# TencentYoutuResearch/ImageMatching-OETR

Hardware: AMD Instinct MI355X
Metric: image-pairs/sec @640x640 (OETR hot path: feature correlation + overlap regression, features resident in HBM) (higher is better)
Workload: dtype f32 (3xf16-split operands, fp32 accumulate); 1 GPU; BASELINE configs[1]: batch=8 pairs/GPU, 640x640 -> 20x20 tokens/image, C=256, 8 enc + 2 dec layers, f32_split_f16; pairs_per_gpu=8, global_pairs=8, streams=3, world_size=1, gpu_max_hw_queues=4, encoder_tile_rows=64, tail_mode=direct form (throughput setting for overlapped streams), parallelism=pairs sharded over 1 rank(s); all-gather of boxes only

## Files before the change

### imagematching_oetr_amd/csrc/api.hip

```cpp
#include <math.h>
#include <stdlib.h>
#include <string.h>

#include <atomic>
#include <string>
#include <vector>

#include "../../include/oetr_hip.h"
#include "../../include/oetr_tail_share.h"
#include "common.h"

using namespace oetr;

constexpr int OETR_PREREDUCE_MIN_TOKENS = 768;
constexpr int OETR_DIRECT_TAIL_MIN_ROWS = 16000;

namespace {

thread_local std::string g_err;

oetr_status fail(oetr_status st, const std::string& msg) {
  g_err = msg;
  return st;
}
// ... 124 lines not shown
  size_t dev_floats = 0;
  EncLayerDev enc[OETR_N_ENC];
  DecKVDev dkv;
  DecLayerDev dec[OETR_N_DEC];
  const float* qe[2];
  const float *dec_tgt1, *dec_q0, *dec_qkv1;
  HeadsDev heads;
};

struct oetr_neck_ctx {
  oetr_trace* trace = nullptr;
  int device = 0;
  int num_cus = 256;
  int conv_rows = 0;
  float* dev = nullptr;
  const f32x4 *proj_wh[2], *proj_wl[2];
  const float *proj_b, *ln_w, *ln_b;
  const f32x4 *conv_wh[3], *conv_wl[3];
  const f32x4 *conv_wh_rw[3], *conv_wl_rw[3];
  int conv_kernel = 0;
  const float* conv_b[3];
  const f32x4 *out_wh, *out_wl;
  const float* out_b;
};

namespace {

#ifdef OETR_PHASE_TIMING
long long* g_tbuf = nullptr;
#endif

struct Workspace {
  float *x, *qp, *pos, *kvp[2], *ksp[2], *att0, *z0, *dkv1, *dks1, *conv_out, *gn_part, *sm_part, *hs,
      *logits, *cxy, *tlbr, *convp, *kbuf[2], *vt[2], *kvr, *ksr;
  uint32_t* flags;
  size_t bytes;
};

bool make_geom(int n, int hf1, int wf1, int hf2, int wf2, Geom* g) {
  if (n <= 0 || hf1 <= 0 || wf1 <= 0 || hf2 <= 0 || wf2 <= 0) return false;
  const long L1 = (long)hf1 * wf1, L2 = (long)hf2 * wf2;
  if (L1 > OETR_MAX_TOKENS || L2 > OETR_MAX_TOKENS) return false;
  if ((long)n * (L1 + L2) > (1L << 30) / C) return false;
  g->N = n;
  g->L[0] = (int)L1; g->L[1] = (int)L2;
  g->hf[0] = hf1; g->wf[0] = wf1; g->hf[1] = hf2; g->wf[1] = wf2;
  g->nt[0] = (g->L[0] + TM - 1) / TM; g->nt[1] = (g->L[1] + TM - 1) / TM;
  g->row0[0] = 0; g->row0[1] = n * g->L[0];
  g->prow0[0] = 0; g->prow0[1] = g->L[0];
  g->tile0[0] = 0; g->tile0[1] = n * g->nt[0];
  g->ntiles = n * (g->nt[0] + g->nt[1]);
  g->rows = n * (g->L[0] + g->L[1]);
  return true;
}

int encoder_tile_rows(const oetr_ctx* h, const Geom& g) {
  if (!gm_half(h->mode) || h->attn_full) return TM;
  const int want = h->enc_tile;
  if (want == TM || want == 64) return want;
  return g.ntiles > h->num_cus ? 64 : TM;
}
Geom encoder_geom(const Geom& g, int rows) {
  Geom e = g;
  for (int i = 0; i < 2; ++i) e.nt[i] = (g.L[i] + rows - 1) / rows;
  e.tile0[0] = 0; e.tile0[1] = g.N * e.nt[0];
  e.ntiles = g.N * (e.nt[0] + e.nt[1]);
  return e;
}

Workspace carve(const Geom& g, void* base, bool attn_full = false) {
  Workspace w;
  size_t off = 0;
  auto take = [&](size_t floats) {
    float* p = base ? reinterpret_cast<float*>(static_cast<char*>(base) + off) : nullptr;
    off += (floats * sizeof(float) + 255) & ~size_t(255);
    return p;
  };
  const size_t rows = g.rows, nt = g.ntiles;
  w.flags = reinterpret_cast<uint32_t*>(take(OETR_WORKSPACE_STATUS_BYTES / sizeof(float)));
  w.x = take(rows * C);
  w.qp = take((rows + (size_t)2 * g.N * 64) * C);
  w.pos = take((size_t)(g.L[0] + g.L[1]) * C);
  for (int i = 0; i < 2; ++i) { w.kvp[i] = take(nt * KV_FLOATS); w.ksp[i] = take(nt * C); }
  w.att0 = take(nt * C); w.z0 = take(nt * NH);
  w.dkv1 = take(nt * KV_FLOATS); w.dks1 = take(nt * C);
  w.conv_out = take(rows * C);
  w.gn_part = take(nt * 32 * 2);
  w.sm_part = take(nt * 4);
  w.hs = take((size_t)2 * g.N * C);
  w.logits = take(rows);
  w.cxy = take((size_t)2 * g.N * 2);
  w.tlbr = take((size_t)2 * g.N * 4);
  w.convp = take((size_t)9 * rows * C);
  w.kvr = take((size_t)2 * g.N * KV_FLOATS);
  w.ksr = take((size_t)2 * g.N * C);
  for (int i = 0; i < 2; ++i) {
    w.kbuf[i] = attn_full ? take(rows * C) : nullptr;
    w.vt[i] = attn_full ? take((size_t)g.N * C * TM * (g.nt[0] + g.nt[1])) : nullptr;
  }
  w.bytes = off;
  return w;
}

oetr_status check_ws(const Geom& g, void* ws, size_t ws_bytes, Workspace* out, bool attn_full = false) {
  if (!ws) return fail(OETR_ERR_WORKSPACE, "workspace is NULL");
  if (reinterpret_cast<uintptr_t>(ws) & 255)
    return fail(OETR_ERR_WORKSPACE, "workspace must be 256-byte aligned");
  *out = carve(g, ws, attn_full);
  if (out->bytes > ws_bytes)
    return fail(OETR_ERR_WORKSPACE, "workspace too small: need " + std::to_string(out->bytes) +
                                        " bytes, got " + std::to_string(ws_bytes));
  return OETR_OK;
}

HeatLaunch heat_launch(const oetr_ctx* h, const Geom& g, const Workspace& w, const float* mem1,
                       const float* mem2, const float* hs1, const float* hs2, float* cxy1,
                       float* cxy2, int img_h1, int img_h2) {
  HeatLaunch p;
  p.g = g;
  p.w = h->heads;
  p.mem[0] = mem1; p.mem[1] = mem2;
  p.hs[0] = hs1; p.hs[1] = hs2;
  p.conv_out = w.conv_out;
  p.gn_part = w.gn_part;
  p.sm_part = w.sm_part;
  p.logits = w.logits;
  p.cxy[0] = cxy1; p.cxy[1] = cxy2;
  p.img_h[0] = img_h1; p.img_h[1] = img_h2;
  p.tlbr[0] = p.tlbr[1] = nullptr;
  p.box[0] = p.box[1] = nullptr;
  p.img_w[0] = p.img_w[1] = 0;
  p.flags = w.flags;
  p.publish = nullptr;
  p.force_staged_conv = h->tail_mode == 3;
  p.convp_units = 9;
  p.mask[0] = p.mask[1] = nullptr;
  return p;
}

oetr_status check_masks(const oetr_ctx* h, const float* mask1, const float* mask2, bool encoder) {
  if (!mask1 && !mask2) return OETR_OK;
  if (!mask1 || !mask2) return fail(OETR_ERR_BAD_ARG, "masks: pass both mask1 and mask2, or neither");
  if (encoder && ((h->mode != GM_SPLIT && h->mode != GM_F32) || h->attn_full))
    return fail(OETR_ERR_UNSUPPORTED, "masks: built for OETR_DTYPE_F32_SPLIT_F16, OETR_DTYPE_F32_SPLIT_QK16 and OETR_DTYPE_F32 with linear attention "
                                      "(the reference's FullAttention turns a masked query row into NaN, "
                                      "linear_attention.py:74-81)");
  return OETR_OK;
}

struct Scoped {
  oetr_trace* t; hipStream_t s; int slot;
  Scoped(oetr_trace* tr, hipStream_t s_, int kid) : t(tr), s(s_), slot(-1) {
    if (!t) return;
    if (2 * (t->used + 1) > (int)t->ev.size()) { t->dropped++; t = nullptr; return; }
    slot = t->used++;
    t->kid[slot] = kid;
    (void)hipEventRecord(t->ev[2 * slot], s);
  }
  ~Scoped() { if (t) (void)hipEventRecord(t->ev[2 * slot + 1], s); }
};
#define TRACED(h, s, kid, expr)            \
  do {                                     \
    Scoped sc__((h)->trace, s, kid);       \
    HIP_TRY(expr);                         \
  } while (0)

DecLaunch dec_launch(const oetr_ctx* h, const Geom& g, const Workspace& w, bool beside_convp = false) {
  DecLaunch d;
  d.g = encoder_geom(g, encoder_tile_rows(h, g));
  for (int i = 0; i < 2; ++i) { d.layer[i] = h->dec[i]; d.qe[i] = h->qe[i]; }
  d.tgt1 = h->dec_tgt1; d.qkv1 = h->dec_qkv1;
  d.att0_part = w.att0; d.z0_part = w.z0; d.dkv1 = w.dkv1; d.dks1 = w.dks1;
  d.hs = w.hs;
  const int images = 2 * g.N;
  bool fits = images <= DEC_SPLIT_MAX_IMAGES && images * DEC_SPLIT_K * 4 <= h->num_cus;
  d.convp_units = 9;
  if (fits && beside_convp) {
    if (gm_half(h->mode)) {
      const int units = 9 * g.N * ((g.L[0] + RT - 1) / RT + (g.L[1] + RT - 1) / RT);
      const int avail = h->num_cus - images * DEC_SPLIT_K;
      const int upi = std::max(3, (units + avail - 1) / avail);
      fits = upi <= 9;
      if (fits) d.convp_units = upi;
    } else {
      fits = images * DEC_SPLIT_K + g.ntiles <= h->num_cus;
    }
  }
  if (h->dec_split == DEC_SPLIT_K && d.convp_units == 9 && beside_convp && gm_half(h->mode)) d.convp_units = 3;
  d.ksplit = (h->dec_split == DEC_SPLIT_K || (h->dec_split == 0 && fits)) && images <= DEC_SPLIT_MAX_IMAGES
                 ? DEC_SPLIT_K : 1;
  d.flags = w.flags;
  d.xch_epoch = w.flags + STATUS_EPOCH_WORD;
  d.xch = reinterpret_cast<unsigned long long*>(reinterpret_cast<char*>(w.flags) + STATUS_XCH_OFFSET);
  d.tbuf = nullptr;
  d.dbg = 0;
  if (d.ksplit == DEC_SPLIT_K && h->dec_fault) { d.dbg = DEC_DBG_FAULT; h->dec_fault = 0; }
#ifdef OETR_PHASE_TIMING
  d.tbuf = g_tbuf ? g_tbuf + 16 * 4096 : nullptr;
#endif
  return d;
}

oetr_status run_correlation(oetr_ctx* h, const Geom& g, const Workspace& w, const float* feat1,
                            const float* feat2, const float* pos1, const float* pos2,
                            int enc_layers, hipStream_t s, bool with_decoder = true,
                            bool resident = false, const float* mask1 = nullptr,
// ... 355 lines not shown
  if (!make_geom(n_pairs, hf1, wf1, hf2, wf2, &g))
    return fail(OETR_ERR_BAD_SHAPE, "invalid shape: need N>0 and 1 <= hf*wf <= " +
                                        std::to_string(OETR_MAX_TOKENS));
  if (full && (img_h1 < hf1 || img_h2 < hf2 || img_w1 <= 0 || img_w2 <= 0))
    return fail(OETR_ERR_BAD_SHAPE, "image size smaller than the token grid");
  Workspace w;
  oetr_status rc = check_ws(g, workspace, workspace_bytes, &w, h->attn_full);
  if (rc) return rc;
  hipStream_t s = static_cast<hipStream_t>(stream);
  rc = run_correlation(h, g, w, feat1, feat2, pos1, pos2, enc_layers, s, false, resident,
                       mask1, mask2);
  if (rc) return rc;
  const size_t r1 = (size_t)g.N * g.L[0], r2 = (size_t)g.N * g.L[1];
  if (st) {
    if ((rc = copy_out(st->memory1, w.x, r1 * C, s))) return rc;
    if ((rc = copy_out(st->memory2, w.x + r1 * C, r2 * C, s))) return rc;
  }
  if (!full) return OETR_OK;
  const float* hs1 = w.hs;
  const float* hs2 = w.hs + (size_t)g.N * C;
  float* cxy1 = w.cxy;
  float* cxy2 = w.cxy + 2 * g.N;
  float* tl1 = w.tlbr;
  float* tl2 = w.tlbr + 4 * g.N;
  HeatLaunch hp = heat_launch(h, g, w, w.x, w.x + r1 * C, hs1, hs2, cxy1, cxy2, img_h1, img_h2);
  hp.tlbr[0] = tl1; hp.tlbr[1] = tl2;
  hp.mask[0] = mask1; hp.mask[1] = mask2;
  hp.box[0] = box1; hp.box[1] = box2;
  hp.img_w[0] = img_w1; hp.img_w[1] = img_w2;
  hp.publish = publish;
  const bool direct = h->mode == GM_SPLIT &&
                      (h->tail_mode >= 2 || (h->tail_mode == 0 && g.rows >= OETR_DIRECT_TAIL_MIN_ROWS));
  if (direct) {
    TRACED(h, s, K_DECODER, launch_decoder(dec_launch(h, g, w), s));
    TRACED(h, s, K_HEAT_CONV, launch_heat_conv64(hp, h->mode, s));
  } else {
    TRACED(h, s, K_DEC_CONVP, launch_decoder_convp(dec_launch(h, g, w, true), hp, w.convp, h->mode, s));
    TRACED(h, s, K_HEAT_COMBINE, launch_heat_combine(hp, w.convp, s));
  }
  TRACED(h, s, K_HEAT_FINAL, launch_heat_final(hp, s));
  if (st) {
    if ((rc = copy_out(st->hs1, hs1, (size_t)g.N * C, s))) return rc;
    if ((rc = copy_out(st->hs2, hs2, (size_t)g.N * C, s))) return rc;
    if ((rc = copy_out(st->logits1, w.logits, r1, s))) return rc;
    if ((rc = copy_out(st->logits2, w.logits + r1, r2, s))) return rc;
    if ((rc = copy_out(st->cxy1, cxy1, 2 * g.N, s))) return rc;
    if ((rc = copy_out(st->cxy2, cxy2, 2 * g.N, s))) return rc;
    if ((rc = copy_out(st->tlbr1, tl1, 4 * g.N, s))) return rc;
    if ((rc = copy_out(st->tlbr2, tl2, 4 * g.N, s))) return rc;
  }
  return OETR_OK;
}
}

oetr_status oetr_forward_stages(oetr_handle h, const float* feat1, const float* feat2,
                                const float* pos1, const float* pos2, int n_pairs, int hf1,
                                int wf1, int hf2, int wf2, int img_h1, int img_w1, int img_h2,
                                int img_w2, void* workspace, size_t workspace_bytes,
                                float* box1, float* box2, const oetr_stage_outputs* st,
                                void* stream) {
  return forward_impl(h, feat1, feat2, pos1, pos2, n_pairs, hf1, wf1, hf2, wf2, img_h1, img_w1,
                      img_h2, img_w2, workspace, workspace_bytes, box1, box2, st, stream, false);
}

oetr_status oetr_forward_masked(oetr_handle h, const float* feat1, const float* feat2,
                                const float* pos1, const float* pos2, const float* mask1,
                                const float* mask2, int n_pairs, int hf1, int wf1, int hf2, int wf2,
// ... 653 lines not shown

oetr_status oetr_trace_summary(oetr_trace_handle t, int* n_kernels,
                               const char* names[OETR_TRACE_MAX_KERNELS],
                               int launches[OETR_TRACE_MAX_KERNELS],
                               float total_ms[OETR_TRACE_MAX_KERNELS]) {
  if (!t || !n_kernels || !names || !launches || !total_ms)
    return fail(OETR_ERR_BAD_ARG, "oetr_trace_summary: NULL argument");
  static_assert(K_COUNT <= OETR_TRACE_MAX_KERNELS, "raise OETR_TRACE_MAX_KERNELS");
  for (int i = 0; i < K_COUNT; ++i) { names[i] = kKernelNames[i]; launches[i] = 0; total_ms[i] = 0.f; }
  for (int i = 0; i < t->used; ++i) {
    HIP_TRY(hipEventSynchronize(t->ev[2 * i + 1]));
    float ms = 0.f;
    HIP_TRY(hipEventElapsedTime(&ms, t->ev[2 * i], t->ev[2 * i + 1]));
    launches[t->kid[i]]++;
    total_ms[t->kid[i]] += ms;
  }
  *n_kernels = K_COUNT;
  const int dropped = t->dropped;
  t->used = 0;
  t->dropped = 0;
  if (dropped) return fail(OETR_ERR_BAD_ARG, std::to_string(dropped) + " launches not traced: pool too small");
  return OETR_OK;
}

#ifdef OETR_PHASE_TIMING
int oetr_debug_read_tbuf(long long* host, int n_blocks) {
  if (!g_tbuf) return 1;
  return hipMemcpy(host, g_tbuf, sizeof(long long) * 16 * n_blocks, hipMemcpyDeviceToHost) != hipSuccess;
}
int oetr_debug_read_tbuf_decoder(long long* host, int n_blocks) {
  if (!g_tbuf) return 1;
  return hipMemcpy(host, g_tbuf + 16 * 4096, sizeof(long long) * 16 * n_blocks, hipMemcpyDeviceToHost) != hipSuccess;
}
#endif

}
```

### imagematching_oetr_amd/csrc/common.h

```cpp
#pragma once
#include <hip/hip_runtime.h>
#include <stdint.h>

#include <string>
#include <type_traits>

#include "../../include/oetr_hip.h"

namespace oetr {

constexpr int C = 256;
constexpr int NH = 8;
constexpr int HD = 32;
constexpr int FF = 512;
constexpr int TM = 32;
constexpr int LDA = C + 4;
constexpr int LDH = FF + 4;
constexpr int NTHREADS = 256;
constexpr int KV_FLOATS = NH * HD * HD;
constexpr float LN_EPS = 1e-5f;
constexpr float ATTN_EPS = 1e-6f;
constexpr int MAX_TOKENS = 10000;


// ... 839 lines not shown
  long long* tbuf;
  uint32_t* flags;
  const float* feat_nchw[2];
  const float* pos_nchw[2];
  float* pos_out;
  const float* mask[2];
};

hipError_t launch_encoder(const EncLaunch& p, bool has_b, int tail, int mode, hipStream_t s);
int encoder_workgroups(const EncLaunch& p, int mode);
hipError_t launch_kv_reduce(const Geom& g, const float* kvp, const float* ksp, float* kvr, float* ksr,
                            hipStream_t s);

struct MhaDev {
  const float *wq_t, *wk_t, *wv_t, *wm_t;
  const float *bq, *bk, *bv;
};
struct DecLayerDev {
  MhaDev self_attn, cross;
  const float *w1_t, *w2_t;
  const float *n1w, *n1b, *n2w, *n2b, *n3w, *n3b;
};
struct DecLaunch {
  Geom g;
  DecLayerDev layer[2];
  const float* qe[2];
  const float* tgt1;
  const float* qkv1;
  const float* att0_part;
  const float* z0_part;
  const float* dkv1;
  const float* dks1;
  float* hs;
  int convp_units;
  int ksplit;
  unsigned long long* xch;
  unsigned* xch_epoch;
  uint32_t* flags;
  long long* tbuf;
  int dbg;
};
struct DecConstLaunch {
  DecLayerDev layer[2];
  const float* qe[2];
  float *tgt1, *q0, *qkv1;
};
hipError_t launch_decoder_consts(const DecConstLaunch& p, hipStream_t s);
hipError_t launch_decoder(const DecLaunch& p, hipStream_t s);

struct HeadsDev {
  const f32x4* conv_w;
  const f32x4* conv_w_l;
  const float *conv_b, *gn_w, *gn_b, *out_w, *out_b;
  const float *tlbr0_t;
  const float *tlbr2_w, *tlbr2_b;
};
struct HeatLaunch {
  Geom g;
  HeadsDev w;
  const float* mem[2];
  const float* hs[2];
  float* conv_out;
  float* gn_part;
  float* sm_part;
  float* logits;
  float* cxy[2];
  int img_h[2];
  float* tlbr[2];
  float* box[2];
  int img_w[2];
  uint32_t* flags;
  uint32_t* publish;
  int force_staged_conv;
  int convp_units;
  const float* mask[2];
};
hipError_t launch_heat_conv(const HeatLaunch& p, int mode, hipStream_t s);
hipError_t launch_heat_conv64(const HeatLaunch& p, int mode, hipStream_t s);
hipError_t launch_decoder_convp(const DecLaunch& d, const HeatLaunch& h, float* P, int mode,
                                hipStream_t s);
hipError_t launch_heat_combine(const HeatLaunch& h, const float* P, hipStream_t s);
hipError_t launch_heat_final(const HeatLaunch& p, hipStream_t s);
hipError_t launch_size_regression(const HeadsDev& w, const float* hs1, const float* hs2,
                                  int n, float* tlbr1, float* tlbr2, hipStream_t s);
hipError_t launch_boxes(const float* cxy, const float* tlbr, int n, int max_h, int max_w,
                        float* box, hipStream_t s);
constexpr int BBC = 1024;
constexpr int NECK_MT = 256;
constexpr int NECK_PIX = 16;
constexpr int NECK_XROW = 2 * C;
constexpr int NECK_RW_MIN_WO = 16;
struct NeckGeom {
  int n_img, hb, wb, ho, wo;
  int HW;
  int rows_in;
  int M;
};
struct NeckProjLaunch {
  NeckGeom g;
  const float* bb;
  const f32x4 *wh[2], *wl[2];
  const float *bias, *ln_w, *ln_b;
  _Float16 *xh, *xl;
  uint32_t* flags;
};
struct NeckConvDesc {
  const f32x4 *wh, *wl;
  const f32x4 *wh_rw, *wl_rw;
// ... 41 lines not shown
```

### imagematching_oetr_amd/csrc/decoder.hip

```cpp
#include "common.h"
#include "conv_p.h"

namespace oetr {

constexpr int DEC_THREADS = 1024;

template <int K, int NOUT>
__device__ __forceinline__ void gemv_partial(const float* __restrict__ Wt, const float* x_s,
                                             float* part_s, int tid) {
  constexpr int NO4 = NOUT / 4;
  constexpr int KCH = DEC_THREADS / NO4;
  constexpr int KPER = K / KCH;
  constexpr int BATCH = KPER < 16 ? KPER : 16;
  const int kc = tid / NO4, o4 = tid % NO4;
  const f32x4* w = reinterpret_cast<const f32x4*>(Wt) + (size_t)kc * KPER * NO4 + o4;
  f32x4 acc = {0.f, 0.f, 0.f, 0.f};
#pragma unroll
  for (int i0 = 0; i0 < KPER; i0 += BATCH) {
    f32x4 wv[BATCH];
#pragma unroll
    for (int i = 0; i < BATCH; ++i) wv[i] = w[(size_t)(i0 + i) * NO4];
#pragma unroll
    for (int i = 0; i < BATCH; ++i) acc += wv[i] * x_s[kc * KPER + i0 + i];
  }
  *reinterpret_cast<f32x4*>(part_s + kc * NOUT + 4 * o4) = acc;
}
template <int K, int NOUT>
__device__ __forceinline__ float gemv_collect(const float* part_s, int o) {
  constexpr int KCH = DEC_THREADS / (NOUT / 4);
  float s = 0.f;
#pragma unroll
  for (int c = 0; c < KCH; ++c) s += part_s[c * NOUT + o];
  return s;
// ... 280 lines not shown
  if (tid < C) vq[tid] = elu1(gemv_get<T, C, C>(part_s, tid) + w1.cross.bq[tid]);
  __syncthreads();
  if (tid < C) {
    const int h = tid >> 5, v = tid & 31;
    float z = 0.f, s = 0.f;
#pragma unroll 4
    for (int d = 0; d < HD; ++d) {
      const float fq = vq[h * HD + d];
      z += fq * ksum[h * HD + d];
      s += fq * kv_s[(h * HD + d) * HD + v];
    }
    att[tid] = s * (1.0f / (z + ATTN_EPS)) * (float)L;
  }
  __syncthreads();
  PHASE_STAMP(p, 7);
  acc = zero4;
  gemv_stage<T, C, C>(w1.cross.wm_t, att, tid, wv, acc, [&] { gemv_issue<T, C, FF, 0>(w1.w1_t, tid, wv); });
  gemv_put<T, C, C>(acc, part_s, tid);
  __syncthreads();
  if (tid < C) tgt[tid] += gemv_get<T, C, C>(part_s, tid);
  __syncthreads();
  PHASE_STAMP(p, 8);
  ln_vec(tgt, w1.n3w, w1.n3b, t2, nullptr, nullptr, tid);
  acc = zero4;
  gemv_stage<T, C, FF>(w1.w1_t, t2, tid, wv, acc, [&] { gemv_issue<T, FF, C, 0>(w1.w2_t, tid, wv); });
  gemv_put<T, C, FF>(acc, part_s, tid);
  __syncthreads();
  for (int o = tid; o < FF; o += T) hdn_s[o] = fmaxf(gemv_get<T, C, FF>(part_s, o), 0.f);
  __syncthreads();
  acc = zero4;
  gemv_stage<T, FF, C>(w1.w2_t, hdn_s, tid, wv, acc, [] {});
  gemv_put<T, FF, C>(acc, part_s, tid);
  __syncthreads();
  if (tid < C) p.hs[(size_t)img * C + tid] = tgt[tid] + gemv_get<T, FF, C>(part_s, tid);
  PHASE_STAMP(p, 9);
}

constexpr int DEC_K = DEC_SPLIT_K;
constexpr int XCH_STAGES = DEC_SPLIT_EXCHANGES;
constexpr long long DEC_SPIN_LIMIT = 200000;

typedef __attribute__((address_space(1))) unsigned long long gu64;

struct DecSmem4 {
  static constexpr int KV = 0, PARTS = KV + 2 * HD * HD, VEC = PARTS + 3 * 2048, SLAB = VEC + 4 * C,
                       TOTAL = SLAB + 64 * 3 + 192 + 128;
};

template <int KS, int B0>
__device__ __forceinline__ void issue_rows(const float* __restrict__ Wt, int j, int tid, f32x4 (&w)[16]) {
  constexpr int KPER = KS / 8;
  const f32x4* src = reinterpret_cast<const f32x4*>(Wt) + (size_t)(j * KS + (tid >> 6) * KPER) * (C / 4) + (tid & 63);
#pragma unroll
  for (int i = 0; i < KPER; ++i) w[B0 + i] = src[i * (C / 4)];
  __builtin_amdgcn_sched_barrier(0);
}
template <int NS, int LD, int B0>
__device__ __forceinline__ void issue_cols(const float* __restrict__ Wt, int j, int tid, f32x4 (&w)[16]) {
  constexpr int NO4 = NS / 4, KCH = 512 / NO4, KPER = C / KCH;
  const f32x4* src = reinterpret_cast<const f32x4*>(Wt) + (size_t)((tid / NO4) * KPER) * (LD / 4) + j * NO4 + tid % NO4;
#pragma unroll
  for (int i = 0; i < KPER; ++i) w[B0 + i] = src[i * (LD / 4)];
  __builtin_amdgcn_sched_barrier(0);
}
template <int KS, int B0>
__device__ __forceinline__ void fma_rows(const f32x4 (&w)[16], const float* x_s, float* part_s, int tid) {
  constexpr int KPER = KS / 8;
  const int kc = tid >> 6;
// ... 173 lines not shown
  PHASE_STAMP(p, 5);
  fma_rows<64, 8>(wa, att, part_s, tid);
  issue_cols<128, FF, 0>(w1.w1_t, j, tid, wa);
  __syncthreads();
  if (tid < C) tgt[tid] += exchange_sum<false>(p, img, 2, j, tag, collect<8, C>(part_s, tid), tid, dead);
  __syncthreads();
  PHASE_STAMP(p, 6);
  ln_vec(tgt, w1.n2w, w1.n2b, t2, qe, qk, tid);
  fma_cols<64, 0>(wb, qk, part_s, tid);
  __syncthreads();
  if (tid < 64) vq[tid] = elu1(collect<32, 64>(part_s, tid) + w1.cross.bq[64 * j + tid]);
  __syncthreads();
  if (tid < 64) {
    const int hl = tid >> 5, v = tid & 31;
    float z = 0.f, sacc = 0.f;
#pragma unroll 4
    for (int d = 0; d < HD; ++d) {
      const float fq = vq[hl * HD + d];
      z += fq * ksum[hl * HD + d];
      sacc += fq * kv_s[(hl * HD + d) * HD + v];
    }
    att[tid] = sacc * (1.0f / (z + ATTN_EPS)) * (float)L;
  }
  __syncthreads();
  PHASE_STAMP(p, 7);
  fma_rows<64, 8>(wb, att, part_s, tid);
  issue_rows<128, 0>(w1.w2_t, j, tid, wb);
  __syncthreads();
  if (tid < C) tgt[tid] += exchange_sum<false>(p, img, 3, j, tag, collect<8, C>(part_s, tid), tid, dead);
  __syncthreads();
  PHASE_STAMP(p, 8);
  ln_vec(tgt, w1.n3w, w1.n3b, t2, nullptr, nullptr, tid);
  fma_cols<128, 0>(wa, t2, part_s, tid);
  __syncthreads();
  if (tid < 128) hdn_s[tid] = fmaxf(collect<16, 128>(part_s, tid), 0.f);
  __syncthreads();
  fma_rows<128, 0>(wb, hdn_s, part_s, tid);
  __syncthreads();
  if (tid < C) {
    const float s = exchange_sum<true>(p, img, 4, j, tag, collect<8, C>(part_s, tid), tid, dead);
    if (j == 0) {
      p.hs[(size_t)img * C + tid] = tgt[tid] + s;
      if (tid == 0) __hip_atomic_store(p.xch_epoch + img, tag, __ATOMIC_RELAXED, __HIP_MEMORY_SCOPE_AGENT);
    }
  }
  PHASE_STAMP(p, 9);
}

constexpr int DEC_WG_THREADS = 512;
template <int T>
__global__ __launch_bounds__(T) void k_decoder(DecLaunch p) {
  __shared__ __attribute__((aligned(16))) float smem[DecSmem<T>::TOTAL];
  decoder_body<T>(p, blockIdx.x, smem);
}
__global__ __launch_bounds__(512) void k_decoder4(DecLaunch p) {
  __shared__ __attribute__((aligned(16))) float smem[DecSmem4::TOTAL];
  decoder_body4(p, blockIdx.x / DEC_K, blockIdx.x % DEC_K, smem);
}

hipError_t launch_decoder(const DecLaunch& p, hipStream_t s) {
  if (p.ksplit == DEC_K)
    hipLaunchKernelGGL(k_decoder4, dim3(2 * p.g.N * DEC_K), dim3(512), 0, s, p);
  else
    hipLaunchKernelGGL(k_decoder<DEC_WG_THREADS>, dim3(2 * p.g.N), dim3(DEC_WG_THREADS), 0, s, p);
  return hipGetLastError();
}

template <int MODE, bool T64>
__global__ __launch_bounds__(512) void k_decoder_convp(DecLaunch d, HeatLaunch h, float* P) {
  constexpr int TILE = T64 ? R_FLOATS : TILE_FLOATS;
  static_assert(DecSmem4::TOTAL <= DecSmem<512>::TOTAL, "decoder LDS");
  constexpr int LDS_FLOATS = DecSmem<512>::TOTAL > TILE ? DecSmem<512>::TOTAL : TILE;
  __shared__ __attribute__((aligned(16))) float smem[LDS_FLOATS];
  const int nd = 2 * d.g.N * d.ksplit;
  if ((int)blockIdx.x < nd) {
    if (d.ksplit == DEC_K) decoder_body4(d, blockIdx.x / DEC_K, blockIdx.x % DEC_K, smem);
    else decoder_body<512>(d, blockIdx.x, smem);
  } else if constexpr (T64) conv_p_body64<MODE>(h, P, blockIdx.x - nd, smem);
  else conv_p_body<MODE>(h, P, blockIdx.x - nd, smem);
// ... 28 lines not shown
```

### imagematching_oetr_amd/csrc/heads.hip

```cpp
#include "common.h"

namespace oetr {

constexpr int GN_GROUPS = 32;
constexpr float GN_EPS = 1e-5f;

template <int MODE, int NW>
__global__ __launch_bounds__(64 * NW) void k_heat_conv(HeatLaunch p) {
  constexpr int NT = 8 / NW, THREADS = 64 * NW, WC = 32 * NT;
  constexpr int TPR = THREADS / TM, F4 = 64 / TPR;
  __shared__ __attribute__((aligned(16))) float smem[2 * TILE_FLOATS];
  const Geom& g = p.g;
  const int tid = threadIdx.x, lane = tid & 63, wave = __builtin_amdgcn_readfirstlane(tid >> 6), half = lane >> 5;
  const int col = lane & 31;

  const int logical = xcd_remap(blockIdx.x, g.ntiles);
  const int per = g.nt[0] + g.nt[1];
  const int n = logical / per;
  const int rem = logical - n * per;
  const int side = rem >= g.nt[0];
  const int t_idx = side ? rem - g.nt[0] : rem;
  const int L = g.L[side], hf = g.hf[side], wf = g.wf[side];
  const int l0 = t_idx * TM;
  const int nvalid = min(TM, L - l0);
// ... 196 lines not shown
    m2 += __shfl_xor(m2, 32, 64);
    if ((lane & 39) == 0) {
      float* dst = p.gn_part + ((size_t)(slot0 + mt) * GN_GROUPS + (c >> 3)) * 2;
      dst[0] = mean;
      dst[1] = m2;
    }
  }
}

template <int MODE, int ROWS>
__device__ __forceinline__ void heat_conv64_body(const HeatLaunch& p, float* smem, float* att_s, float* attmax_s) {
  static_assert(gm_planes(MODE) == 2, "two-plane mode");
  static_assert(16 % WStream2T<MODE, ROWS>::D == 0, "tap loop below assumes a ring phase of 0 after every GEMM");
  constexpr int THREADS = 512, TPR = THREADS / RT, F4 = 64 / TPR;
  const Geom& g = p.g;
  const int tid = threadIdx.x, lane = tid & 63, wave = __builtin_amdgcn_readfirstlane(tid >> 6);
  const int half = lane >> 5, col = lane & 31;
  const int nt0 = (g.L[0] + RT - 1) / RT, nt1 = (g.L[1] + RT - 1) / RT;
  const int logical = xcd_remap(blockIdx.x, g.N * (nt0 + nt1));
  const int per = nt0 + nt1;
  const int n = logical / per;
  const int rem = logical - n * per;
  const int side = rem >= nt0;
  const int t_idx = side ? rem - nt0 : rem;
  const int L = g.L[side], hf = g.hf[side], wf = g.wf[side];
  const int l0 = t_idx * RT;
  const int nvalid = min(RT, L - l0);
  const float* mem = p.mem[side] + (size_t)n * L * C;
  const size_t row_base = (size_t)g.row0[side] + (size_t)n * L + l0;
  Range rg;
  const int halo0 = l0 - wf - 1, nhalo = RT + 2 * (wf + 1);
  const int hrow = tid / TPR, hpart = tid % TPR;
  {
    const f32x4* hsp = reinterpret_cast<const f32x4*>(p.hs[side] + (size_t)n * C) + hpart;
    f32x4 hv[F4];
#pragma unroll
    for (int i = 0; i < F4; ++i) hv[i] = hsp[i * TPR];
    for (int r0 = 0; r0 < nhalo; r0 += RT) {
      const int hr = r0 + hrow;
      const int l = min(max(halo0 + hr, 0), L - 1);
      const f32x4* mp = reinterpret_cast<const f32x4*>(mem + (size_t)l * C) + hpart;
      float d = 0.f;
#pragma unroll
      for (int i = 0; i < F4; ++i) {
        const f32x4 v = mp[i * TPR];
        d += (v[0] * hv[i][0] + v[1] * hv[i][1]) + (v[2] * hv[i][2] + v[3] * hv[i][3]);
      }
      d = sum8(d);
      if (hpart == 0 && hr < nhalo) att_s[hr] = d;
    }
  }
  __syncthreads();
  {
    float m = 0.f;
    for (int i = tid; i < nhalo; i += THREADS) m = fmaxf(m, fabsf(att_s[i]));
    m = wave_max(m);
    if (lane == 0) attmax_s[wave] = m;
  }
  __syncthreads();
  float att_scale = 1.0f, att_unscale = 1.0f;
  {
    float m = attmax_s[0];
#pragma unroll
    for (int i = 1; i < THREADS / 64; ++i) m = fmaxf(m, attmax_s[i]);
    if (m > 0.f && m < INFINITY) {
      const int e = ilogbf(m) + 1;
      att_scale = ldexpf(1.0f, -e);
      att_unscale = ldexpf(1.0f, e);
    }
  }
  auto region = [&](int t) { return PlanesT<MODE>(smem + (t & 1) * R_FLOATS, &rg); };
  const int lrow = l0 + hrow;
  const int y = lrow / wf, x = lrow - y * wf;
  auto tap_loads = [&](int tap, f32x4 (&v)[F4], float& att) {
    const int dy = tap / 3 - 1, dx = tap % 3 - 1;
    const int yy = y + dy, xx = x + dx;
    const bool ok = (lrow < L) && (yy >= 0) && (yy < hf) && (xx >= 0) && (xx < wf);
    const int src_row = ok ? yy * wf + xx : 0;
    att = ok ? att_s[src_row - halo0] * att_scale : 0.f;
    const f32x4* mp = reinterpret_cast<const f32x4*>(mem + (size_t)src_row * C) + hpart;
#pragma unroll
    for (int i = 0; i < F4; ++i) v[i] = mp[i * TPR];
  };
// ... 34 lines not shown
#pragma unroll
  for (int mt = 0; mt < 2; ++mt)
#pragma unroll
    for (int r = 0; r < 16; ++r) acc[mt][r] = fmaf(acc[mt][r], att_unscale, bias);
  range_report<MODE>(rg, p.flags);

  heat_conv64_finish(p, acc, g, side, n, t_idx, nvalid, row_base, lane, wave, half, col);
}

constexpr int HALO_MAX_WF = 40;
constexpr int HALO_MAX_ROWS = RT + 2 * (HALO_MAX_WF + 1);
template <int MODE, int ROWS>
__device__ __forceinline__ void heat_conv64h_body(const HeatLaunch& p, _Float16* planes, float* att_s, float* mask_s,
                                                  float* attmax_s) {
  static_assert(gm_planes(MODE) == 2, "two-plane mode");
  static_assert(16 % WStream2T<MODE, ROWS>::D == 0, "the tap sequence below assumes a ring phase of 0 after every GEMM");
  constexpr int THREADS = 512, TPR = THREADS / RT, F4 = 64 / TPR;
  const Geom& g = p.g;
  const int tid = threadIdx.x, lane = tid & 63, wave = __builtin_amdgcn_readfirstlane(tid >> 6);
  const int half = lane >> 5, col = lane & 31;
  const int nt0 = (g.L[0] + RT - 1) / RT, nt1 = (g.L[1] + RT - 1) / RT;
  const int logical = xcd_remap(blockIdx.x, g.N * (nt0 + nt1));
  const int per = nt0 + nt1;
  const int n = logical / per;
  const int rem = logical - n * per;
  const int side = rem >= nt0;
  const int t_idx = side ? rem - nt0 : rem;
  const int L = g.L[side], wf = g.wf[side];
  const int l0 = t_idx * RT;
  const int nvalid = min(RT, L - l0);
  const float* mem = p.mem[side] + (size_t)n * L * C;
  const size_t row_base = (size_t)g.row0[side] + (size_t)n * L + l0;
  Range rg;
  const int halo0 = l0 - wf - 1, nhalo = RT + 2 * (wf + 1);
  const int hrow = tid / TPR, hpart = tid % TPR;
  constexpr int NPASS = (HALO_MAX_ROWS + RT - 1) / RT;
  f32x4 hv[F4];
  {
    const f32x4* hsp = reinterpret_cast<const f32x4*>(p.hs[side] + (size_t)n * C) + hpart;
#pragma unroll
    for (int i = 0; i < F4; ++i) hv[i] = hsp[i * TPR];
  }
#pragma unroll 1
  for (int ps = 0; ps < NPASS; ++ps) {
    const int hr = ps * RT + hrow;
    const int l = min(max(halo0 + hr, 0), L - 1);
    const f32x4* mp = reinterpret_cast<const f32x4*>(mem + (size_t)l * C) + hpart;
    float d = 0.f;
#pragma unroll
    for (int i = 0; i < F4; ++i) {
      const f32x4 v = mp[i * TPR];
      d += (v[0] * hv[i][0] + v[1] * hv[i][1]) + (v[2] * hv[i][2] + v[3] * hv[i][3]);
    }
    d = sum8(d);
    if (hpart == 0 && hr < nhalo) att_s[hr] = d;
  }
  if (tid < RT) {
    const int l = l0 + tid, x = l - (l / wf) * wf;
    mask_s[tid] = x != 0 ? 1.0f : 0.0f;
    mask_s[RT + tid] = x != wf - 1 ? 1.0f : 0.0f;
  }
  __syncthreads();
  {
    float m = 0.f;
    for (int i = tid; i < nhalo; i += THREADS) m = fmaxf(m, fabsf(att_s[i]));
    m = wave_max(m);
    if (lane == 0) attmax_s[wave] = m;
  }
  __syncthreads();
  float att_scale = 1.0f, att_unscale = 1.0f;
  {
    float m = attmax_s[0];
#pragma unroll
    for (int i = 1; i < THREADS / 64; ++i) m = fmaxf(m, attmax_s[i]);
    if (m > 0.f && m < INFINITY) {
      const int e = ilogbf(m) + 1;
      att_scale = ldexpf(1.0f, -e);
      att_unscale = ldexpf(1.0f, e);
    }
  }
  _Float16* const hi0 = planes;
  _Float16* const lo0 = planes + HALO_MAX_ROWS * LDAH;
  WStream2T<MODE, ROWS> ws;
  ws.set_rows(nvalid);
  ws.set_lane(lane);
  constexpr size_t TAP_UNITS = (size_t)C * C / 8;
  auto tap_of = [](int k) { return 3 * (k % 3) + k / 3; };
  ws.template prime<C, 0>(p.w.conv_w + tap_of(0) * TAP_UNITS, p.w.conv_w_l + tap_of(0) * TAP_UNITS, wave, 0, lane);
  {
    const PlanesT<MODE> H(hi0, lo0, &rg);
#pragma unroll 1
    for (int ps = 0; ps < NPASS; ++ps) {
      const int hr = ps * RT + hrow;
      if (hr < nhalo) {
        const int l = halo0 + hr;
        const bool in = l >= 0 && l < L;
        const float att = in ? att_s[hr] * att_scale : 0.f;
        const f32x4* mp = reinterpret_cast<const f32x4*>(mem + (size_t)min(max(l, 0), L - 1) * C) + hpart;
#pragma unroll
        for (int i = 0; i < F4; ++i) H.put4(hr, 4 * (i * TPR + hpart), mp[i * TPR] * att);
      }
    }
  }
  __syncthreads();
  f32x16 acc[2] = {f32x16{0}, f32x16{0}}, accR[2] = {f32x16{0}, f32x16{0}};
  auto window = [&](int k) {
    const int dy = k % 3 - 1, dx = k / 3 - 1;
    const int shift = (wf + 1) + dy * wf + dx;
    return PlanesT<MODE>(hi0 + shift * LDAH, lo0 + shift * LDAH, &rg);
  };
  auto run = [&](int k, f32x16 (&a)[2], auto HAS_NEXT_) {
    constexpr bool HAS_NEXT = decltype(HAS_NEXT_)::value;
    const int t = tap_of(k), tn = tap_of(HAS_NEXT ? k + 1 : k);
    ws.template gemm<C, 0, HAS_NEXT, C>(window(k), p.w.conv_w + t * TAP_UNITS, p.w.conv_w_l + t * TAP_UNITS, wave, 0, lane,
                                        a, p.w.conv_w + tn * TAP_UNITS, p.w.conv_w_l + tn * TAP_UNITS, wave, 0);
  };
#pragma unroll 1
  for (int k = 0; k < 3; ++k) run(k, acc, std::true_type{});
#pragma unroll
  for (int mt = 0; mt < 2; ++mt)
#pragma unroll
    for (int r = 0; r < 16; ++r) acc[mt][r] *= mask_s[32 * mt + crow(r, half)];
#pragma unroll 1
  for (int k = 3; k < 6; ++k) run(k, acc, std::true_type{});
#pragma unroll 1
  for (int k = 6; k < 8; ++k) run(k, accR, std::true_type{});
  run(8, accR, std::false_type{});
  const float bias = p.w.conv_b[32 * wave + col];
#pragma unroll
  for (int mt = 0; mt < 2; ++mt)
#pragma unroll
    for (int r = 0; r < 16; ++r)
      acc[mt][r] = fmaf(fmaf(accR[mt][r], mask_s[RT + 32 * mt + crow(r, half)], acc[mt][r]), att_unscale, bias);
  range_report<MODE>(rg, p.flags);
  heat_conv64_finish(p, acc, g, side, n, t_idx, nvalid, row_base, lane, wave, half, col);
}

template <int MODE>
__global__ __launch_bounds__(512) void k_heat_conv64(HeatLaunch p) {
  __shared__ __attribute__((aligned(16))) float smem[2 * R_FLOATS];
  __shared__ float att_s[RT + 2 * (100 + 1) + 6];
  __shared__ float attmax_s[512 / 64];
  const Geom& g = p.g;
  const int nt0 = (g.L[0] + RT - 1) / RT, nt1 = (g.L[1] + RT - 1) / RT;
  if ((int)blockIdx.x >= g.N * (nt0 + nt1)) return size_reg_body(p, blockIdx.x - g.N * (nt0 + nt1), smem);
  const int logical = xcd_remap(blockIdx.x, g.N * (nt0 + nt1));
  const int rem = logical - (logical / (nt0 + nt1)) * (nt0 + nt1);
  const int side = rem >= nt0;
  const int t_idx = side ? rem - nt0 : rem;
  const int nvalid = min(RT, g.L[side] - t_idx * RT);
  if (__builtin_amdgcn_readfirstlane(nvalid > 32 ? 1 : 0)) heat_conv64_body<MODE, 2>(p, smem, att_s, attmax_s);
  else heat_conv64_body<MODE, 1>(p, smem, att_s, attmax_s);
}

template <int MODE>
__global__ __launch_bounds__(512) void k_heat_conv64h(HeatLaunch p) {
  __shared__ __attribute__((aligned(16))) _Float16 planes[2 * HALO_MAX_ROWS * LDAH];
  __shared__ float att_s[HALO_MAX_ROWS + 6];
  __shared__ float mask_s[2 * RT];
  __shared__ float attmax_s[512 / 64];
  const Geom& g = p.g;
  const int nt0 = (g.L[0] + RT - 1) / RT, nt1 = (g.L[1] + RT - 1) / RT;
  if ((int)blockIdx.x >= g.N * (nt0 + nt1))
    return size_reg_body(p, blockIdx.x - g.N * (nt0 + nt1), reinterpret_cast<float*>(planes));
  const int logical = xcd_remap(blockIdx.x, g.N * (nt0 + nt1));
  const int rem = logical - (logical / (nt0 + nt1)) * (nt0 + nt1);
  const int side = rem >= nt0;
  const int t_idx = side ? rem - nt0 : rem;
// ... 326 lines not shown
```

Before: 34590 image-pairs/s.

## Compute attention dot products in decoder tail and reuse them in heat conv

```diff
diff --git a/imagematching_oetr_amd/csrc/api.hip b/imagematching_oetr_amd/csrc/api.hip
--- a/imagematching_oetr_amd/csrc/api.hip
+++ b/imagematching_oetr_amd/csrc/api.hip
@@ -180,7 +180,7 @@
 
 struct Workspace {
   float *x, *qp, *pos, *kvp[2], *ksp[2], *att0, *z0, *dkv1, *dks1, *conv_out, *gn_part, *sm_part, *hs,
-      *logits, *cxy, *tlbr, *convp, *kbuf[2], *vt[2], *kvr, *ksr;
+      *logits, *cxy, *tlbr, *convp, *kbuf[2], *vt[2], *kvr, *ksr, *att;
   uint32_t* flags;
   size_t bytes;
 };
@@ -246,6 +246,7 @@
     w.kbuf[i] = attn_full ? take(rows * C) : nullptr;
     w.vt[i] = attn_full ? take((size_t)g.N * C * TM * (g.nt[0] + g.nt[1])) : nullptr;
   }
+  w.att = take(rows);
   w.bytes = off;
   return w;
 }
@@ -269,6 +270,7 @@
   p.w = h->heads;
   p.mem[0] = mem1; p.mem[1] = mem2;
   p.hs[0] = hs1; p.hs[1] = hs2;
+  p.att = w.att;
   p.conv_out = w.conv_out;
   p.gn_part = w.gn_part;
   p.sm_part = w.sm_part;
@@ -283,6 +285,10 @@
   p.force_staged_conv = h->tail_mode == 3;
   p.convp_units = 9;
   p.mask[0] = p.mask[1] = nullptr;
+  p.tbuf = nullptr;
+#ifdef OETR_PHASE_TIMING
+  p.tbuf = g_tbuf ? g_tbuf + 16 * 8192 : nullptr;
+#endif
   return p;
 }
 
@@ -320,6 +326,7 @@
   d.tgt1 = h->dec_tgt1; d.qkv1 = h->dec_qkv1;
   d.att0_part = w.att0; d.z0_part = w.z0; d.dkv1 = w.dkv1; d.dks1 = w.dks1;
   d.hs = w.hs;
+  d.mem[0] = d.mem[1] = nullptr; d.att = nullptr;
   const int images = 2 * g.N;
   bool fits = images <= DEC_SPLIT_MAX_IMAGES && images * DEC_SPLIT_K * 4 <= h->num_cus;
   d.convp_units = 9;
@@ -741,7 +748,9 @@
   const bool direct = h->mode == GM_SPLIT &&
                       (h->tail_mode >= 2 || (h->tail_mode == 0 && g.rows >= OETR_DIRECT_TAIL_MIN_ROWS));
   if (direct) {
-    TRACED(h, s, K_DECODER, launch_decoder(dec_launch(h, g, w), s));
+    DecLaunch dl = dec_launch(h, g, w);
+    dl.mem[0] = hp.mem[0]; dl.mem[1] = hp.mem[1]; dl.att = w.att;
+    TRACED(h, s, K_DECODER, launch_decoder(dl, s));
     TRACED(h, s, K_HEAT_CONV, launch_heat_conv64(hp, h->mode, s));
   } else {
     TRACED(h, s, K_DEC_CONVP, launch_decoder_convp(dec_launch(h, g, w, true), hp, w.convp, h->mode, s));
@@ -1461,6 +1470,10 @@
   if (!g_tbuf) return 1;
   return hipMemcpy(host, g_tbuf + 16 * 4096, sizeof(long long) * 16 * n_blocks, hipMemcpyDeviceToHost) != hipSuccess;
 }
+int oetr_debug_read_tbuf_heat(long long* host, int n_blocks) {
+  if (!g_tbuf) return 1;
+  return hipMemcpy(host, g_tbuf + 16 * 8192, sizeof(long long) * 16 * n_blocks, hipMemcpyDeviceToHost) != hipSuccess;
+}
 #endif
 
 }
diff --git a/imagematching_oetr_amd/csrc/att_dot.h b/imagematching_oetr_amd/csrc/att_dot.h
--- /dev/null
+++ b/imagematching_oetr_amd/csrc/att_dot.h
@@ -0,0 +1,61 @@
+#pragma once
+#include "common.h"
+
+namespace oetr {
+
+constexpr int ATT_TPR = 8;
+constexpr int ATT_F4 = 64 / ATT_TPR;
+
+__device__ __forceinline__ void att_load(const float* row, int part, f32x4 (&v)[ATT_F4]) {
+  const f32x4* src = reinterpret_cast<const f32x4*>(row) + part;
+#pragma unroll
+  for (int i = 0; i < ATT_F4; ++i) v[i] = src[i * ATT_TPR];
+}
+
+__device__ __forceinline__ float att_dot(const f32x4 (&v)[ATT_F4], const f32x4 (&hv)[ATT_F4]) {
+#pragma clang fp contract(off)
+  float d = 0.f;
+#pragma unroll
+  for (int i = 0; i < ATT_F4; ++i) {
+    const float a = __builtin_fmaf(v[i][0], hv[i][0], v[i][1] * hv[i][1]);
+    const float b = __builtin_fmaf(v[i][2], hv[i][2], v[i][3] * hv[i][3]);
+    d += a + b;
+  }
+  return sum8(d);
+}
+
+template <int NT>
+__device__ __forceinline__ void att_rows_issue(const float* __restrict__ mem, int r, int r1, int tid,
+                                               f32x4 (&v)[2][ATT_F4]) {
+  constexpr int RP = NT / ATT_TPR;
+  const int row = tid / ATT_TPR, part = tid % ATT_TPR;
+  if (r >= r1) return;
+  att_load(mem + (size_t)min(r + row, r1 - 1) * C, part, v[0]);
+  att_load(mem + (size_t)min(r + RP + row, r1 - 1) * C, part, v[1]);
+}
+template <int NT>
+__device__ __forceinline__ void att_rows_finish(const f32x4 (&v)[2][ATT_F4], const f32x4 (&hv)[ATT_F4],
+                                                float* __restrict__ att, int r, int r1, int tid) {
+  constexpr int RP = NT / ATT_TPR;
+  const int row = tid / ATT_TPR, part = tid % ATT_TPR;
+  if (r >= r1) return;
+  const int ra = r + row, rb = r + RP + row;
+  const float da = att_dot(v[0], hv), db = att_dot(v[1], hv);
+  if (part == 0 && ra < r1) att[ra] = da;
+  if (part == 0 && rb < r1) att[rb] = db;
+}
+template <int NT>
+__device__ __forceinline__ void att_rows(const float* __restrict__ mem, const float* hs, float* __restrict__ att,
+                                         int r0, int r1, int tid) {
+  if (r0 >= r1) return;
+  f32x4 hv[ATT_F4];
+  att_load(hs, tid % ATT_TPR, hv);
+#pragma unroll 1
+  for (int r = r0; r < r1; r += 2 * (NT / ATT_TPR)) {
+    f32x4 v[2][ATT_F4];
+    att_rows_issue<NT>(mem, r, r1, tid, v);
+    att_rows_finish<NT>(v, hv, att, r, r1, tid);
+  }
+}
+
+}
diff --git a/imagematching_oetr_amd/csrc/common.h b/imagematching_oetr_amd/csrc/common.h
--- a/imagematching_oetr_amd/csrc/common.h
+++ b/imagematching_oetr_amd/csrc/common.h
@@ -895,6 +895,8 @@
   const float* dkv1;
   const float* dks1;
   float* hs;
+  const float* mem[2];
+  float* att;
   int convp_units;
   int ksplit;
   unsigned long long* xch;
@@ -923,6 +925,7 @@
   HeadsDev w;
   const float* mem[2];
   const float* hs[2];
+  const float* att;
   float* conv_out;
   float* gn_part;
   float* sm_part;
@@ -937,6 +940,7 @@
   int force_staged_conv;
   int convp_units;
   const float* mask[2];
+  long long* tbuf;
 };
 hipError_t launch_heat_conv(const HeatLaunch& p, int mode, hipStream_t s);
 hipError_t launch_heat_conv64(const HeatLaunch& p, int mode, hipStream_t s);
diff --git a/imagematching_oetr_amd/csrc/decoder.hip b/imagematching_oetr_amd/csrc/decoder.hip
--- a/imagematching_oetr_amd/csrc/decoder.hip
+++ b/imagematching_oetr_amd/csrc/decoder.hip
@@ -1,4 +1,5 @@
 #include "common.h"
+#include "att_dot.h"
 #include "conv_p.h"
 
 namespace oetr {
@@ -345,8 +346,12 @@
   gemv_stage<T, FF, C>(w1.w2_t, hdn_s, tid, wv, acc, [] {});
   gemv_put<T, FF, C>(acc, part_s, tid);
   __syncthreads();
-  if (tid < C) p.hs[(size_t)img * C + tid] = tgt[tid] + gemv_get<T, FF, C>(part_s, tid);
+  if (tid < C) t2[tid] = p.hs[(size_t)img * C + tid] = tgt[tid] + gemv_get<T, FF, C>(part_s, tid);
   PHASE_STAMP(p, 9);
+  if (p.att) {
+    __syncthreads();
+    att_rows<T>(p.mem[side] + (size_t)n * L * C, t2, p.att + g.row0[side] + (size_t)n * L, 0, L, tid);
+  }
 }
 
 constexpr int DEC_K = DEC_SPLIT_K;
@@ -586,19 +591,37 @@
   PHASE_STAMP(p, 8);
   ln_vec(tgt, w1.n3w, w1.n3b, t2, nullptr, nullptr, tid);
   fma_cols<128, 0>(wa, t2, part_s, tid);
+  const bool with_att = p.att != nullptr;
+  const int att_chunk = (L + DEC_K - 1) / DEC_K;
+  const int att_r0 = with_att ? min(j * att_chunk, L) : 0, att_r1 = with_att ? min((j + 1) * att_chunk, L) : 0;
+  const float* att_mem = with_att ? p.mem[side] + (size_t)n * L * C : nullptr;
+  f32x4 av[2][ATT_F4];
+  att_rows_issue<T>(att_mem, att_r0, att_r1, tid, av);
+  __builtin_amdgcn_sched_barrier(0);
   __syncthreads();
   if (tid < 128) hdn_s[tid] = fmaxf(collect<16, 128>(part_s, tid), 0.f);
   __syncthreads();
   fma_rows<128, 0>(wb, hdn_s, part_s, tid);
   __syncthreads();
   if (tid < C) {
-    const float s = exchange_sum<true>(p, img, 4, j, tag, collect<8, C>(part_s, tid), tid, dead);
+    const float mine = collect<8, C>(part_s, tid);
+    const float s = with_att ? exchange_sum<false>(p, img, 4, j, tag, mine, tid, dead)
+                             : exchange_sum<true>(p, img, 4, j, tag, mine, tid, dead);
+    t2[tid] = tgt[tid] + s;
     if (j == 0) {
-      p.hs[(size_t)img * C + tid] = tgt[tid] + s;
+      p.hs[(size_t)img * C + tid] = t2[tid];
       if (tid == 0) __hip_atomic_store(p.xch_epoch + img, tag, __ATOMIC_RELAXED, __HIP_MEMORY_SCOPE_AGENT);
     }
   }
   PHASE_STAMP(p, 9);
+  if (with_att) {
+    __syncthreads();
+    float* att_img = p.att + g.row0[side] + (size_t)n * L;
+    f32x4 hv[ATT_F4];
+    att_load(t2, tid % ATT_TPR, hv);
+    att_rows_finish<T>(av, hv, att_img, att_r0, att_r1, tid);
+    att_rows<T>(att_mem, t2, att_img, att_r0 + 2 * (T / ATT_TPR), att_r1, tid);
+  }
 }
 
 constexpr int DEC_WG_THREADS = 512;
diff --git a/imagematching_oetr_amd/csrc/heads.hip b/imagematching_oetr_amd/csrc/heads.hip
--- a/imagematching_oetr_amd/csrc/heads.hip
+++ b/imagematching_oetr_amd/csrc/heads.hip
@@ -252,23 +252,9 @@
   const int halo0 = l0 - wf - 1, nhalo = RT + 2 * (wf + 1);
   const int hrow = tid / TPR, hpart = tid % TPR;
   {
-    const f32x4* hsp = reinterpret_cast<const f32x4*>(p.hs[side] + (size_t)n * C) + hpart;
-    f32x4 hv[F4];
-#pragma unroll
-    for (int i = 0; i < F4; ++i) hv[i] = hsp[i * TPR];
-    for (int r0 = 0; r0 < nhalo; r0 += RT) {
-      const int hr = r0 + hrow;
-      const int l = min(max(halo0 + hr, 0), L - 1);
-      const f32x4* mp = reinterpret_cast<const f32x4*>(mem + (size_t)l * C) + hpart;
-      float d = 0.f;
-#pragma unroll
-      for (int i = 0; i < F4; ++i) {
-        const f32x4 v = mp[i * TPR];
-        d += (v[0] * hv[i][0] + v[1] * hv[i][1]) + (v[2] * hv[i][2] + v[3] * hv[i][3]);
-      }
-      d = sum8(d);
-      if (hpart == 0 && hr < nhalo) att_s[hr] = d;
-    }
+    const float* att_img = p.att + (size_t)g.row0[side] + (size_t)n * L;
+    for (int hr = tid; hr < nhalo; hr += THREADS)
+      att_s[hr] = att_img[min(max(halo0 + hr, 0), L - 1)];
   }
   __syncthreads();
   {
@@ -369,52 +355,15 @@
   const float* mem = p.mem[side] + (size_t)n * L * C;
   const size_t row_base = (size_t)g.row0[side] + (size_t)n * L + l0;
   Range rg;
+  PHASE_STAMP(p, 0);
   const int halo0 = l0 - wf - 1, nhalo = RT + 2 * (wf + 1);
   const int hrow = tid / TPR, hpart = tid % TPR;
-  constexpr int NPASS = (HALO_MAX_ROWS + RT - 1) / RT;
-  f32x4 hv[F4];
-  {
-    const f32x4* hsp = reinterpret_cast<const f32x4*>(p.hs[side] + (size_t)n * C) + hpart;
-#pragma unroll
-    for (int i = 0; i < F4; ++i) hv[i] = hsp[i * TPR];
-  }
-#pragma unroll 1
-  for (int ps = 0; ps < NPASS; ++ps) {
-    const int hr = ps * RT + hrow;
-    const int l = min(max(halo0 + hr, 0), L - 1);
-    const f32x4* mp = reinterpret_cast<const f32x4*>(mem + (size_t)l * C) + hpart;
-    float d = 0.f;
-#pragma unroll
-    for (int i = 0; i < F4; ++i) {
-      const f32x4 v = mp[i * TPR];
-      d += (v[0] * hv[i][0] + v[1] * hv[i][1]) + (v[2] * hv[i][2] + v[3] * hv[i][3]);
-    }
-    d = sum8(d);
-    if (hpart == 0 && hr < nhalo) att_s[hr] = d;
-  }
+  const float* att_img = p.att + (size_t)g.row0[side] + (size_t)n * L;
+  const float att_mine = att_img[min(max(halo0 + min(tid, nhalo - 1), 0), L - 1)];
   if (tid < RT) {
     const int l = l0 + tid, x = l - (l / wf) * wf;
     mask_s[tid] = x != 0 ? 1.0f : 0.0f;
     mask_s[RT + tid] = x != wf - 1 ? 1.0f : 0.0f;
-  }
-  __syncthreads();
-  {
-    float m = 0.f;
-    for (int i = tid; i < nhalo; i += THREADS) m = fmaxf(m, fabsf(att_s[i]));
-    m = wave_max(m);
-    if (lane == 0) attmax_s[wave] = m;
-  }
-  __syncthreads();
-  float att_scale = 1.0f, att_unscale = 1.0f;
-  {
-    float m = attmax_s[0];
-#pragma unroll
-    for (int i = 1; i < THREADS / 64; ++i) m = fmaxf(m, attmax_s[i]);
-    if (m > 0.f && m < INFINITY) {
-      const int e = ilogbf(m) + 1;
-      att_scale = ldexpf(1.0f, -e);
-      att_unscale = ldexpf(1.0f, e);
-    }
   }
   _Float16* const hi0 = planes;
   _Float16* const lo0 = planes + HALO_MAX_ROWS * LDAH;
@@ -424,22 +373,50 @@
   constexpr size_t TAP_UNITS = (size_t)C * C / 8;
   auto tap_of = [](int k) { return 3 * (k % 3) + k / 3; };
   ws.template prime<C, 0>(p.w.conv_w + tap_of(0) * TAP_UNITS, p.w.conv_w_l + tap_of(0) * TAP_UNITS, wave, 0, lane);
-  {
+  float att_unscale = 1.0f;
+  auto stage = [&](auto NP_) {
+    constexpr int NP = decltype(NP_)::value;
+    f32x4 v[NP][F4];
+#pragma unroll
+    for (int ps = 0; ps < NP; ++ps) {
+      const int l = min(max(halo0 + ps * RT + hrow, 0), L - 1);
+      const f32x4* mp = reinterpret_cast<const f32x4*>(mem + (size_t)l * C) + hpart;
+#pragma unroll
+      for (int i = 0; i < F4; ++i) v[ps][i] = mp[i * TPR];
+    }
+    if (tid < nhalo) att_s[tid] = att_mine;
+    const float m = wave_max(tid < nhalo ? fabsf(att_mine) : 0.f);
+    if (lane == 0) attmax_s[wave] = m;
+    __syncthreads();
+    float att_scale = 1.0f;
+    {
+      float mx = attmax_s[0];
+#pragma unroll
+      for (int i = 1; i < THREADS / 64; ++i) mx = fmaxf(mx, attmax_s[i]);
+      if (mx > 0.f && mx < INFINITY) {
+        const int e = ilogbf(mx) + 1;
+        att_scale = ldexpf(1.0f, -e);
+        att_unscale = ldexpf(1.0f, e);
+      }
+    }
     const PlanesT<MODE> H(hi0, lo0, &rg);
-#pragma unroll 1
-    for (int ps = 0; ps < NPASS; ++ps) {
+#pragma unroll
+    for (int ps = 0; ps < NP; ++ps) {
       const int hr = ps * RT + hrow;
       if (hr < nhalo) {
         const int l = halo0 + hr;
         const bool in = l >= 0 && l < L;
         const float att = in ? att_s[hr] * att_scale : 0.f;
-        const f32x4* mp = reinterpret_cast<const f32x4*>(mem + (size_t)min(max(l, 0), L - 1) * C) + hpart;
-#pragma unroll
-        for (int i = 0; i < F4; ++i) H.put4(hr, 4 * (i * TPR + hpart), mp[i * TPR] * att);
+#pragma unroll
+        for (int i = 0; i < F4; ++i) H.put4(hr, 4 * (i * TPR + hpart), v[ps][i] * att);
       }
     }
-  }
-  __syncthreads();
+  };
+  static_assert(HALO_MAX_ROWS <= 3 * RT, "three passes hold the widest halo");
+  if (nhalo <= 2 * RT) stage(std::integral_constant<int, 2>{});
+  else stage(std::integral_constant<int, 3>{});
+  __syncthreads();
+  PHASE_STAMP(p, 1);
   f32x16 acc[2] = {f32x16{0}, f32x16{0}}, accR[2] = {f32x16{0}, f32x16{0}};
   auto window = [&](int k) {
     const int dy = k % 3 - 1, dx = k / 3 - 1;
@@ -463,6 +440,7 @@
 #pragma unroll 1
   for (int k = 6; k < 8; ++k) run(k, accR, std::true_type{});
   run(8, accR, std::false_type{});
+  PHASE_STAMP(p, 2);
   const float bias = p.w.conv_b[32 * wave + col];
 #pragma unroll
   for (int mt = 0; mt < 2; ++mt)
@@ -471,6 +449,7 @@
       acc[mt][r] = fmaf(fmaf(accR[mt][r], mask_s[RT + 32 * mt + crow(r, half)], acc[mt][r]), att_unscale, bias);
   range_report<MODE>(rg, p.flags);
   heat_conv64_finish(p, acc, g, side, n, t_idx, nvalid, row_base, lane, wave, half, col);
+  PHASE_STAMP(p, 3);
 }
 
 template <int MODE>
```

New measurement: 34510 image-pairs/s. Within noise of the previous version (-0.2%).
